# vfmatzkin/ct-unet

Hardware: AMD Instinct MI355X
Metric: voxels/sec fwd+bwd, 128^3 fp32 patch (higher is better)
Workload: dtype f32

## Files before the change

ct-unet_amd/csrc/conv3d.hip:

```cpp
#include "common.h"
#include "pack.h"
#include "bn_tail.h"

#ifndef CTU_K3S_OCC
#define CTU_K3S_OCC 2
#endif
#ifndef CTU_K3S_ALL
#define CTU_K3S_ALL 1
#endif
#ifndef CTU_WG_OCC
#define CTU_WG_OCC 2
#endif
#ifndef CTU_WG_BLOCKS
#define CTU_WG_BLOCKS 512
#endif

namespace {

typedef float gv2f __attribute__((ext_vector_type(2)));

struct ConvP {
    const float* in;
    const float* in_scale;
    const float* in_shift;
    const float* wp;
    const float* bias;
    float* out;
    float* stats;
    int in_cs, rin_p, in_relu, out_cs, nout_p, nbias;
    int N, D, H, W;
    int tiles_d, tiles_h, tiles_w;
    int n16;
    ctu_bn_tail tail;
};


__host__ __device__ inline void pick_tile(int W, int* td, int* th, int* tw) {
    if (W >= 16) { *td = 4; *th = 4; *tw = 16; }
    else if (W >= 8) { *td = 4; *th = 8; *tw = 8; }
    else { *td = 4; *th = 4; *tw = 4; }
}



template <int KS, int NT, int TD, int TH, int TW, int CCH = 1>
__global__ __launch_bounds__(256) void conv3d_fwd_kernel(ConvP p) {
    constexpr int PAD = (KS - 1) / 2;
    constexpr int HD = TD + KS - 1, HH = TH + KS - 1, HW = TW + KS - 1;
    constexpr int HV = HD * HH * HW;
    constexpr int NVOX = TD * TH * TW;
    constexpr int NMT = NVOX / 16;
    static_assert(NMT % 4 == 0, "block tile must hold a multiple of 4 M-tiles");
    constexpr int MT = NMT / 4;
    constexpr int STAPS = Taps<KS>::STAPS, NSTAGE = Taps<KS>::NSTAGE;
    constexpr int WFL = STAPS * NT * 128;
    constexpr int VSL = 8 * CCH + 4;
    constexpr int AQ = 2 * CCH;
    constexpr int AITEMS = HV * AQ;
    constexpr int AITER = (AITEMS + 255) / 256;
    static_assert(CCH == 1 || NSTAGE == 1, "multi-chunk staging needs all taps' weights in LDS at once");

    __shared__ __attribute__((aligned(16))) float sA[HV * VSL];
    __shared__ __attribute__((aligned(16))) float sW[CCH * WFL];
    __shared__ float sRed[4 * NT * 16 * 2];

    const int tid = threadIdx.x;
    const int lane = tid & 63, wave = tid >> 6;
// ... 1468 lines not shown
    int kw;
    bool ok = true;
    if (SM == 1 && SN == 1) kw = q;
    else if (SM == 2 && SN == 2) { kw = sm + sn; ok = !(sm == 0 && sn == 1); }
    else if (SN == 2) { if (q == 0) { kw = 0; ok = sn == 0; } else kw = 1 + sn; }
    else { if (q == 0) kw = sm; else { kw = 2; ok = sm == 1; } }
    const int cig = pair % n_ci_g, cog = pair / n_ci_g;
    const int cip = cig * CM + cil, co = cog * CN + col;
    const int ci = (cip < cin_p) ? (cinv ? cinv[cip] : (cip < Ci ? cip : -1)) : -1;
    if (ok && ci >= 0 && co < Co) dw[((size_t)co * Ci + ci) * 27 + r * 3 + kw] = tot;
}

struct K3sGeom { int sm, sn, tw, ntiles, n_ci_g, pairs, gx, tpb, nmf; };
static K3sGeom k3s_geom(int N, int D, int H, int W, int cin_p, int cout_p) {
    K3sGeom g;
    g.sm = cin_p == 8 ? 2 : 1; g.sn = cout_p == 8 ? 2 : 1;
    g.tw = (g.sm == 2 && g.sn == 2) ? 16 : 8;
    g.nmf = (g.sm == 2 && g.sn == 2) ? 9 : ((g.sm == 1 && g.sn == 1) ? 27 : 18);
    g.ntiles = N * ceil_div(D, 4) * ceil_div(H, 4) * ceil_div(W, g.tw);
    g.n_ci_g = ceil_div(cin_p, 16 / g.sm);
    g.pairs = g.n_ci_g * ceil_div(cout_p, 16 / g.sn);
    g.gx = wgrad_gx(g.ntiles, g.pairs);
    if (g.ntiles / g.gx < 4) {
        g.gx = (CTU_WG_BLOCKS / 2) / g.pairs;
        if (g.gx < 1) g.gx = 1;
        if (g.gx > g.ntiles) g.gx = g.ntiles;
    }
    g.tpb = ceil_div(g.ntiles, g.gx);
    g.gx = ceil_div(g.ntiles, g.tpb);
    return g;
}

static bool k3s_lazy_ok(int D, int H, int W, int k, int cin_p, int cout_p) {
    if (!use_k3s(k, W, cin_p, cout_p)) return false;
    const int sm = cin_p == 8 ? 2 : 1, sn = cout_p == 8 ? 2 : 1, tw = (sm == 2 && sn == 2) ? 16 : 8;
    return D % 4 == 0 && H % 4 == 0 && W % tw == 0 && cin_p % (16 / sm) == 0 && cout_p % (16 / sn) == 0;
}

template <int SM, int SN>
static int launch_wgrad_k3s(WgP p, float* dw, int Co, int Ci, const int32_t* cinv, hipStream_t st) {
    const K3sGeom g = k3s_geom(p.N, p.D, p.H, p.W, p.cin_p, p.cout_p);
    p.tiles_d = ceil_div(p.D, 4); p.tiles_h = ceil_div(p.H, 4); p.tiles_w = ceil_div(p.W, g.tw);
    p.ntiles = g.ntiles;
    p.n_ci_t = g.n_ci_g;
    if (p.lz_y) conv3d_wgrad_k3s_kernel<SM, SN, 0, true><<<dim3(g.gx, g.pairs), 256, 0, st>>>(p, g.tpb);
    else conv3d_wgrad_k3s_kernel<SM, SN><<<dim3(g.gx, g.pairs), 256, 0, st>>>(p, g.tpb);
    CTU_CHECK_LAUNCH("conv3d_wgrad_k3s");
    conv3d_wgrad_k3s_reduce_kernel<SM, SN><<<dim3(ceil_div(g.nmf * 256, 64), g.pairs), 64 * RPARTS, 0, st>>>(
        p.ws, dw, Co, Ci, cinv, p.cin_p, p.n_ci_t, g.gx);
    CTU_CHECK_LAUNCH("conv3d_wgrad_k3s_reduce");
    return CTU_OK;
}

template <int SM, int SN>
__global__ __launch_bounds__(256, 2) void conv3d_wgrad_k5s_kernel(WgP p, int tiles_per_block) {
    constexpr int UP = 0, PAD = 2;
    const int kd = blockIdx.z;
    constexpr int TD = 4, TH = 4, TW = (SM == 2 && SN == 2) ? 16 : 8, HD = TD, HH = TH + 2 * PAD, HW = TW + 2 * PAD, HV = HD * HH * HW;
    constexpr int KPR = TW / 4, NKS = TH * KPR;
    constexpr int CM = 16 / SM, CN = 16 / SN;
    constexpr int GW = TW + (SN - 1), GV = TD * TH * GW;
    constexpr int QN = (SM == 2 && SN == 2) ? 2 : ((SM == 1 && SN == 1) ? 5 : (SN == 2 ? 4 : 3));
    constexpr int NMF = 5 * QN;
    constexpr int AQ = CM / 4, GQ = CN / 4;
    constexpr int AITEMS = HV * AQ, AITER = (AITEMS + 255) / 256;
    constexpr int GITEMS = GV * GQ, GITER = (GITEMS + 255) / 256;

    constexpr int SAF = AITER * 256 * 4, SGF = GITER * 256 * 4;
    static_assert(SAF >= HV * CM && SGF >= GV * CN, "stage size");
    __shared__ __attribute__((aligned(16))) float sA[2 * SAF];
    __shared__ __attribute__((aligned(16))) float sG[2 * SGF];

    const int tid = threadIdx.x, lane = tid & 63, wave = tid >> 6;
    const int i = lane & 15, kq = lane >> 4;
    const int cig = blockIdx.y % p.n_ci_t, cog = UP ? (blockIdx.y / p.n_ci_t) % p.n_co_t : blockIdx.y / p.n_ci_t;
    const int par = UP ? blockIdx.y / (p.n_ci_t * p.n_co_t) : 0;
    const int pz = UP == 2 ? (par >> 1) & 1 : (par >> 2) & 1, py = UP == 2 ? par & 1 : (par >> 1) & 1, px = UP == 2 ? 0 : par & 1;
    const int gH = UP ? 2 * p.H : p.H, gW = UP ? 2 * p.W : p.W, gs = UP ? 2 : 1;
    const int ci0 = cig * CM, co0 = cog * CN;
    const bool has_xf = p.in_scale != nullptr;

    f32x4 acc[NMF];
#pragma unroll
    for (int t = 0; t < NMF; ++t) acc[t] = f32x4{0.f, 0.f, 0.f, 0.f};

    const int aq = tid % AQ, gq = tid % GQ;
    const bool a_ok = (ci0 + aq * 4) < p.cin_p, g_ok = (co0 + gq * 4) < p.cout_p;
    float4 sc = make_float4(1.f, 1.f, 1.f, 1.f), sh = make_float4(0.f, 0.f, 0.f, 0.f);
    if (has_xf && a_ok) {
        sc = *reinterpret_cast<const float4*>(p.in_scale + ci0 + aq * 4);
        sh = *reinterpret_cast<const float4*>(p.in_shift + ci0 + aq * 4);
    }
    const int xf_relu = has_xf ? p.in_relu : 0;
    const int boff = (SN == 2) ? ((i < 8) ? i : i - 16) : i;

    int tile = blockIdx.x * tiles_per_block;
    const int tile_end = min(p.ntiles, tile + tiles_per_block);
    float4 va[AITER], vg[GITER];

    unsigned aoff[AITER], goff[GITER];
    constexpr int FPW = 5;
    unsigned fw[(AITER + FPW - 1) / FPW], gw0 = 0;
#pragma unroll
    for (int q = 0; q < (AITER + FPW - 1) / FPW; ++q) fw[q] = 0;
#pragma unroll
    for (int it = 0; it < AITER; ++it) {
// ... 339 lines not shown
        g.tpb = ceil_div(g.ntiles, g.gx);
        g.gx = ceil_div(g.ntiles, g.tpb);
        return g;
    }
    g.nmf = 8;
    g.ntiles = N * ceil_div(D, 4) * ceil_div(H, 4) * ceil_div(W, 8);
    g.n_ci_g = ceil_div(cin_p, 16);
    g.n_co_g = ceil_div(nout_p, 16);
    g.pairs = 8 * g.n_ci_g * g.n_co_g;
    g.gx = wgrad_gx(g.ntiles, g.pairs);
    if (g.ntiles / g.gx < 4) {
        g.gx = (CTU_WG_BLOCKS / 2) / g.pairs;
        if (g.gx < 1) g.gx = 1;
        if (g.gx > g.ntiles) g.gx = g.ntiles;
    }
    g.tpb = ceil_div(g.ntiles, g.gx);
    g.gx = ceil_div(g.ntiles, g.tpb);
    return g;
}

}

static bool use_persist5(int k, int nt, int tw, int N, int D, int H, int W) {
    return k == 5 && tw == 16 && nt <= 2 && (long)N * ceil_div(D, 4) * ceil_div(H, 4) * ceil_div(W, 16) >= 256;
}

extern "C" int ctu_conv3d_layout(int k, int nout_p, int W) {
    return ((k == 3 || k == 5) && nout_p == 8 && W >= 32) ? 1 : 0;
}

extern "C" const char* ctu_conv3d_fwd_kernel_name(int N, int D, int H, int W, int k, int nout_p, int layout) {
    static thread_local char buf[64];
    if (layout == 1) return k == 3 ? "conv3d_fwd_k3_persist<1, true>" : "conv3d_fwd_k5_persist<1, true>";
    int nt, td, th, tw;
    pick_launch(N, D, H, W, k, nout_p, &nt, &td, &th, &tw);
    if (use_persist5(k, nt, tw, N, D, H, W)) snprintf(buf, sizeof(buf), "conv3d_fwd_k5_persist<%d, false>", nt);
    else if (k == 3 && tw == 16 && nt <= 2) snprintf(buf, sizeof(buf), "conv3d_fwd_k3_persist<%d, false>", nt);
    else snprintf(buf, sizeof(buf), "conv3d_fwd_kernel<%d, %d, %d, %d, %d>", k, nt, td, th, tw);
    return buf;
}

extern "C" const char* ctu_conv3d_wgrad_kernel_name(int W, int k, int cin_p, int cout_p) {
    static thread_local char buf[64];
    if (use_k3s(k, W, cin_p, cout_p))
        snprintf(buf, sizeof(buf), "conv3d_wgrad_k3s_kernel<%d, %d>", cin_p == 8 ? 2 : 1, cout_p == 8 ? 2 : 1);
    else if (use_k5s(k, W, cin_p, cout_p))
        snprintf(buf, sizeof(buf), "conv3d_wgrad_k5s_kernel<%d, %d>", cin_p == 8 ? 2 : 1, cout_p == 8 ? 2 : 1);
    else {
        int td, th, tw;
        pick_tile(W, &td, &th, &tw);
        snprintf(buf, sizeof(buf), "conv3d_wgrad_kernel<%d, %d, %d, %d, %d>", k, k == 3 ? 3 : 1, td, th, tw);
    }
    return buf;
}

extern "C" size_t ctu_conv3d_packed_floats(int k, int rin_p, int nout_p, int layout) {
    if ((k != 3 && k != 5) || rin_p <= 0 || nout_p <= 0) return 0;
    if (layout == 1) return nout_p == 8 ? (size_t)(rin_p / 8) * k * k * (k + 1) * 128 : 0;
    return (size_t)(rin_p / 8) * k * k * k * ceil_div(nout_p, 16) * 128;
}

static void persist_grid(int ntiles, int ny, int blocks_per_cu, int* gx, int* tpb) {
    int g = (256 * blocks_per_cu) / ny;
    if (g < 1) g = 1;
    if (g > ntiles) g = ntiles;
    *tpb = ceil_div(ntiles, g);
    *gx = ceil_div(ntiles, *tpb);
}

static bool use_persist(int k, int nt, int tw) { return k == 3 && tw == 16 && nt <= 2; }

extern "C" int ctu_conv3d_num_blocks(int N, int D, int H, int W, int k, int nout_p, int layout) {
    int gx, tpb;
    if (layout == 1) {
        persist_grid(N * ceil_div(D, 4) * ceil_div(H, 4) * ceil_div(W, 32), 1, k == 3 ? 2 : 1, &gx, &tpb);
        return gx;
    }
    int nt, td, th, tw;
    pick_launch(N, D, H, W, k, nout_p, &nt, &td, &th, &tw);
    const int ntiles = N * ceil_div(D, td) * ceil_div(H, th) * ceil_div(W, tw);
    if (use_persist5(k, nt, tw, N, D, H, W)) {
        persist_grid(ntiles, ceil_div(ceil_div(nout_p, 16), nt), 1, &gx, &tpb);
        return gx;
    }
    if (use_persist(k, nt, tw)) {
        persist_grid(ntiles, ceil_div(ceil_div(nout_p, 16), nt), nt == 1 ? CTU_FWD_OCC1 : 2, &gx, &tpb);
        return gx;
    }
    return ntiles;
}

extern "C" int ctu_pack_conv3d_weight(const float* w, float* wp, int Co, int Ci, int k, const int32_t* cinv,
                                      int rin_p, int nout_p, int mode, int layout, void* stream) {
    CTU_REQUIRE(k == 3 || k == 5, "pack_conv3d_weight: k=%d unsupported (3 or 5)", k);
    CTU_REQUIRE(rin_p % 8 == 0 && nout_p % 8 == 0, "pack_conv3d_weight: padded channels must be multiples of 8");
    CTU_REQUIRE(w && wp && Co > 0 && Ci > 0, "pack_conv3d_weight: null/empty argument");
    CTU_REQUIRE(layout == 0 || (layout == 1 && nout_p == 8), "pack_conv3d_weight: layout %d needs nout_p=8", layout);
    hipStream_t st = (hipStream_t)stream;
    if (layout == 1) {
        const int tot = (int)ctu_conv3d_packed_floats(k, rin_p, nout_p, 1);
        if (k == 3) pack_conv_w_pair8_kernel<3><<<ceil_div(tot, 256), 256, 0, st>>>(w, wp, Co, Ci, cinv, rin_p / 8, mode);
        else pack_conv_w_pair8_kernel<5><<<ceil_div(tot, 256), 256, 0, st>>>(w, wp, Co, Ci, cinv, rin_p / 8, mode);
        CTU_CHECK_LAUNCH("pack_conv3d_weight(pair8)");
        return CTU_OK;
    }
    const int n16 = ceil_div(nout_p, 16);
// ... 183 lines not shown
}

struct LazyBn { const float* y; const float* scale; const float* shift; const float* coef; float* out; int cp; };

static int conv3d_wgrad_impl(const float* in, int in_cs, int cin_p, const float* in_scale, const float* in_shift,
                             int in_relu, const float* gout, int g_cs, int cout_p, float* dw, float* dbias, int Co,
                             int Ci, const int32_t* cinv, float* ws, int N, int D, int H, int W, int k, const LazyBn* lz,
                             void* stream);

extern "C" int ctu_conv3d_wgrad(const float* in, int in_cs, int cin_p, const float* in_scale, const float* in_shift,
                                int in_relu, const float* gout, int g_cs, int cout_p, float* dw, float* dbias, int Co,
                                int Ci, const int32_t* cinv, float* ws, int N, int D, int H, int W, int k,
                                void* stream) {
    return conv3d_wgrad_impl(in, in_cs, cin_p, in_scale, in_shift, in_relu, gout, g_cs, cout_p, dw, dbias, Co, Ci, cinv, ws,
                             N, D, H, W, k, nullptr, stream);
}

extern "C" int ctu_conv3d_wgrad_bn_supported(int N, int D, int H, int W, int k, int cin_p, int cout_p) {
    return (N > 0 && k3s_lazy_ok(D, H, W, k, cin_p, cout_p)) ? 1 : 0;
}

extern "C" int ctu_conv3d_wgrad_bn(const float* in, int in_cs, int cin_p, const float* in_scale, const float* in_shift,
                                   int in_relu, const float* ga, int g_cs, int cout_p, const float* y,
                                   const float* bn_scale, const float* bn_shift, const float* coef, float* gy_out,
                                   float* dw, int Co, int Ci, const int32_t* cinv, float* ws, int N, int D, int H, int W,
                                   int k, void* stream) {
    CTU_REQUIRE(y && bn_scale && bn_shift && coef && gy_out, "conv3d_wgrad_bn: null pointer");
    CTU_REQUIRE(k3s_lazy_ok(D, H, W, k, cin_p, cout_p), "conv3d_wgrad_bn: geometry not supported (ask ctu_conv3d_wgrad_bn_supported)");
    CTU_REQUIRE(((uintptr_t)y & 15) == 0 && ((uintptr_t)gy_out & 15) == 0 && gy_out != ga, "conv3d_wgrad_bn: y / gy_out alignment, gy_out must not alias ga");
    const LazyBn lz = {y, bn_scale, bn_shift, coef, gy_out, cout_p};
    return conv3d_wgrad_impl(in, in_cs, cin_p, in_scale, in_shift, in_relu, ga, g_cs, cout_p, dw, nullptr, Co, Ci, cinv, ws,
                             N, D, H, W, k, &lz, stream);
}

static int conv3d_wgrad_impl(const float* in, int in_cs, int cin_p, const float* in_scale, const float* in_shift,
                             int in_relu, const float* gout, int g_cs, int cout_p, float* dw, float* dbias, int Co,
                             int Ci, const int32_t* cinv, float* ws, int N, int D, int H, int W, int k, const LazyBn* lz,
                             void* stream) {
    CTU_REQUIRE(k == 3 || k == 5, "conv3d_wgrad: k=%d unsupported (3 or 5)", k);
    CTU_REQUIRE(in && gout && dw && ws, "conv3d_wgrad: null pointer");
    CTU_REQUIRE(cin_p % 8 == 0 && cout_p % 8 == 0 && cin_p > 0 && cout_p > 0, "conv3d_wgrad: padded channels");
    CTU_REQUIRE(in_cs >= cin_p && in_cs % 4 == 0 && g_cs >= cout_p && g_cs % 4 == 0, "conv3d_wgrad: bad stride");
    CTU_REQUIRE(Co <= cout_p && Co > 0 && Ci > 0 && cin_p <= 256, "conv3d_wgrad: Co/Ci");
    CTU_REQUIRE(((uintptr_t)in & 15) == 0 && ((uintptr_t)gout & 15) == 0, "conv3d_wgrad: 16-byte alignment");
    hipStream_t st = (hipStream_t)stream;
    WgP p;
    p.in = in; p.in_scale = in_scale; p.in_shift = in_shift; p.g = gout; p.ws = ws;
    p.in_cs = in_cs; p.cin_p = cin_p; p.in_relu = in_relu; p.g_cs = g_cs; p.cout_p = cout_p;
    p.N = N; p.D = D; p.H = H; p.W = W;
    p.lz_y = nullptr; p.lz_out = nullptr; p.lz_scale = nullptr; p.lz_shift = nullptr; p.lz_coef = nullptr; p.lz_cp = 0;
    if (lz) { p.lz_y = lz->y; p.lz_out = lz->out; p.lz_scale = lz->scale; p.lz_shift = lz->shift; p.lz_coef = lz->coef; p.lz_cp = lz->cp; }
    int gz, gx, bt;
    wgrad_geom(N, D, H, W, k, cin_p, cout_p, &p.ntiles, &p.n_ci_t, &p.n_co_t, &gz, &gx, &bt);
    if (use_k3s(k, W, cin_p, cout_p)) {
        int rc2;
        if (cin_p == 8 && cout_p == 8) rc2 = launch_wgrad_k3s<2, 2>(p, dw, Co, Ci, cinv, st);
        else if (cout_p == 8) rc2 = launch_wgrad_k3s<1, 2>(p, dw, Co, Ci, cinv, st);
        else if (cin_p == 8) rc2 = launch_wgrad_k3s<2, 1>(p, dw, Co, Ci, cinv, st);
        else rc2 = launch_wgrad_k3s<1, 1>(p, dw, Co, Ci, cinv, st);
        if (rc2 != CTU_OK) return rc2;
        if (dbias) return ctu_channel_sum(gout, g_cs, cout_p, (int64_t)N * D * H * W, ws, dbias, Co, stream);
        return CTU_OK;
    }
    if (use_k5s(k, W, cin_p, cout_p)) {
        CTU_REQUIRE((int64_t)((4 + 2 * 2) * H + 8) * W * in_cs * 4 < (int64_t)1 << 31, "conv3d_wgrad: volume too large for 32-bit offsets");
        int rc2;
        if (cin_p == 8 && cout_p == 8) rc2 = launch_wgrad_k5s<2, 2>(p, dw, Co, Ci, cinv, st);
        else if (cout_p == 8) rc2 = launch_wgrad_k5s<1, 2>(p, dw, Co, Ci, cinv, st);
        else rc2 = launch_wgrad_k5s<2, 1>(p, dw, Co, Ci, cinv, st);
        if (rc2 != CTU_OK) return rc2;
        if (dbias) return ctu_channel_sum(gout, g_cs, cout_p, (int64_t)N * D * H * W, ws, dbias, Co, stream);
        return CTU_OK;
    }
    int rc = (k == 3) ? launch_wgrad<3, 3>(p, dw, Co, Ci, cinv, gz, gx, st)
                      : launch_wgrad<5, 1>(p, dw, Co, Ci, cinv, gz, gx, st);
    if (rc != CTU_OK) return rc;
    if (dbias) return ctu_channel_sum(gout, g_cs, cout_p, (int64_t)N * D * H * W, ws, dbias, Co, stream);
    return CTU_OK;
}

extern "C" size_t ctu_upconv_fused_wgrad_ws_floats(int N, int D, int H, int W, int cin_p, int nout_p) {
    const UpWgGeom a = upwg_geom(N, D, H, W, cin_p, nout_p, false), b = upwg_geom(N, D, H, W, cin_p, nout_p, true);
    const size_t na = (size_t)a.pairs * a.gx * a.nmf * 256, nb = (size_t)b.pairs * b.gx * b.nmf * 256;
    return na > nb ? na : nb;
}

static int upconv_fused_wgrad_impl(const float* in, int in_cs, int cin_p, const float* in_scale, const float* in_shift,
                                   int in_relu, const float* gout, int g_cs, int nout_p, float* dweff, float* ws,
                                   int N, int D, int H, int W, const LazyBn* lz, void* stream);

extern "C" int ctu_upconv_fused_wgrad(const float* in, int in_cs, int cin_p, const float* in_scale, const float* in_shift,
                                      int in_relu, const float* gout, int g_cs, int nout_p, float* dweff, float* ws,
                                      int N, int D, int H, int W, void* stream) {
    return upconv_fused_wgrad_impl(in, in_cs, cin_p, in_scale, in_shift, in_relu, gout, g_cs, nout_p, dweff, ws, N, D, H, W,
                                   nullptr, stream);
}

extern "C" int ctu_upconv_fused_wgrad_bn_supported(int N, int D, int H, int W, int cin_p, int nout_p) {
    return (N > 0 && D % 4 == 0 && H % 4 == 0 && W % 8 == 0 && cin_p % 16 == 0 && nout_p % 8 == 0) ? 1 : 0;
}

extern "C" int ctu_upconv_fused_wgrad_bn(const float* in, int in_cs, int cin_p, const float* in_scale, const float* in_shift,
                                         int in_relu, const float* ga, int g_cs, int nout_p, const float* y,
                                         const float* bn_scale, const float* bn_shift, const float* coef, float* gy_out,
                                         float* dweff, float* ws, int N, int D, int H, int W, void* stream) {
    CTU_REQUIRE(y && bn_scale && bn_shift && coef && gy_out, "upconv_fused_wgrad_bn: null pointer");
// ... 44 lines not shown
```

ct-unet_amd/ctunet_amd/_lib.py:

```python
from __future__ import annotations

import ctypes as C
import os

_HERE = os.path.dirname(os.path.abspath(__file__))
LIB_PATH = os.environ.get("CTUNET_HIP_LIB") or os.path.join(_HERE, "libctunet_hip.so")

P = C.c_void_p
I = C.c_int
L = C.c_int64
F = C.c_float
D = C.c_double
Z = C.c_size_t
U = C.c_uint64

class PackJob(C.Structure):
    _fields_ = [("w", C.c_void_p), ("wp", C.c_void_p), ("cinv", C.c_void_p), ("kind", C.c_int), ("Co", C.c_int),
                ("Ci", C.c_int), ("k", C.c_int), ("rin_p", C.c_int), ("nout_p", C.c_int), ("mode", C.c_int),
                ("layout", C.c_int)]


class BnTail(C.Structure):
    _fields_ = [("gamma", C.c_void_p), ("beta", C.c_void_p), ("running_mean", C.c_void_p), ("running_var", C.c_void_p),
                ("scale", C.c_void_p), ("shift", C.c_void_p), ("mean", C.c_void_p), ("invstd", C.c_void_p),
                ("num_batches_tracked", C.c_void_p), ("counter", C.c_void_p), ("count", C.c_double),
                ("momentum", C.c_float), ("eps", C.c_float), ("C", C.c_int), ("n_updates", C.c_int)]


class BnBwdTail(C.Structure):
    _fields_ = [("gamma", C.c_void_p), ("invstd", C.c_void_p), ("dgamma", C.c_void_p), ("dbeta", C.c_void_p),
                ("coef", C.c_void_p), ("mean", C.c_void_p), ("running_mean", C.c_void_p), ("running_var", C.c_void_p),
                ("num_batches_tracked", C.c_void_p), ("counter", C.c_void_p), ("count", C.c_double),
                ("momentum", C.c_float), ("eps", C.c_float), ("C", C.c_int)]


SIGNATURES = {
    "ctu_last_error": (C.c_char_p, []),
    "ctu_abi_version": (I, []),
    "ctu_arch": (C.c_char_p, []),
    "ctu_ncdhw_to_ndhwc": (I, [P, P, I, I, I, I, I, I, I, P]),
    "ctu_ndhwc_to_ncdhw": (I, [P, P, I, I, I, I, I, I, P]),
    "ctu_conv3d_layout": (I, [I, I, I]),
    "ctu_conv3d_fwd_kernel_name": (C.c_char_p, [I, I, I, I, I, I, I]),
    "ctu_conv3d_wgrad_kernel_name": (C.c_char_p, [I, I, I, I]),
    "ctu_conv3d_packed_floats": (Z, [I, I, I, I]),
    "ctu_conv3d_num_blocks": (I, [I, I, I, I, I, I, I]),
    "ctu_pack_conv3d_weight": (I, [P, P, I, I, I, P, I, I, I, I, P]),
    "ctu_pack_batch": (I, [P, I, P]),
    "ctu_conv3d_fwd": (I, [P, I, I, P, P, I, P, P, I, P, I, I, P, I, I, I, I, I, I, P, P]),
    "ctu_conv3d_wgrad_ws_floats": (Z, [I, I, I, I, I, I, I]),
    "ctu_conv3d_wgrad": (I, [P, I, I, P, P, I, P, I, I, P, P, I, I, P, P, I, I, I, I, I, P]),
    "ctu_conv3d_wgrad_bn_supported": (I, [I, I, I, I, I, I, I]),
    "ctu_conv3d_wgrad_bn": (I, [P, I, I, P, P, I, P, I, I, P, P, P, P, P, P, I, I, P, P, I, I, I, I, I, P]),
    "ctu_conv3d_first_supported": (I, [I, I, I, I]),
    "ctu_conv3d_first_num_blocks": (I, [I, I, I, I]),
    "ctu_conv3d_first_fwd": (I, [P, I, P, P, I, P, I, I, P, I, I, I, I, P, P]),
    "ctu_conv3d_first_bwd_data": (I, [P, I, P, I, I, P, I, I, I, I, P]),
    "ctu_conv3d_first_wgrad_ws_floats": (Z, [I, I, I, I, I]),
    "ctu_conv3d_first_wgrad": (I, [P, I, P, I, P, I, P, I, I, I, I, P]),
    "ctu_conv3d_first_wgrad_bn": (I, [P, I, P, I, P, P, P, P, P, P, I, P, I, I, I, I, P]),
    "ctu_bn_finalize": (I, [P, I, I, I, D, P, P, P, P, F, F, I, P, P, P, P, P, P]),
    "ctu_bn_eval_affine": (I, [P, P, P, P, F, I, I, P, P, P]),
    "ctu_bn_bwd_num_blocks": (I, [L]),
    "ctu_bn_relu_bwd_reduce": (I, [P, I, P, I, I, P, P, P, P, L, P, P, P]),
    "ctu_bn_bwd_finalize": (I, [P, I, I, I, D, P, P, P, P, P, P, P, P, F, F, P, P]),
    "ctu_bn_relu_bwd_apply": (I, [P, I, P, I, I, P, P, P, P, P, L, P]),
    "ctu_maxpool2_fwd": (I, [P, I, I, P, P, I, P, I, I, I, I, I, P]),
    "ctu_maxpool2_bwd": (I, [P, I, I, P, P, I, P, I, P, I, I, I, I, I, I, P]),
    "ctu_maxpool2_bwd_bn_num_blocks": (I, [I, I, I, I, I]),
    "ctu_maxpool2_bwd_bn": (I, [P, I, I, P, P, P, P, P, I, P, I, I, I, I, I, I, P, P, P]),
    "ctu_convt_packed_floats": (Z, [I, I]),
    "ctu_pack_convt_weight": (I, [P, P, I, I, P, I, I, I, P]),
    "ctu_convt2_fwd": (I, [P, I, I, P, P, I, P, P, I, P, I, I, I, I, I, I, P]),
    "ctu_convt2_bwd_data": (I, [P, I, I, P, P, I, I, I, I, I, I, P]),
    "ctu_convt2_wgrad_ws_floats": (Z, [I, I, I, I, I, I]),
    "ctu_convt2_wgrad": (I, [P, I, I, P, P, I, P, I, I, P, P, I, I, P, P, I, I, I, I, P]),
    "ctu_head_fwd": (I, [P, I, I, P, P, I, P, P, P, I, I, I, I, P, P, I, L, P]),
    "ctu_head_bwd_ws_floats": (Z, [I, L, I, I]),
    "ctu_head_bwd": (I, [P, I, I, P, P, I, P, P, P, I, I, I, I, P, P, P, I, P, P, P, I, L, P]),
    "ctu_head_bwd_num_blocks": (I, [I, L]),
    "ctu_head_bwd_bn": (I, [P, I, I, P, P, I, P, P, P, I, I, I, I, P, P, P, I, P, P, P, I, L, P, P, I, P, P, P]),
    "ctu_loss_ws_floats": (Z, [I, L]),
    "ctu_loss_fwd": (I, [P, P, I, L, F, F, I, P, P, P]),
    "ctu_loss_bwd": (I, [P, P, I, L, F, F, I, P, P, P, P, I, P]),
    "ctu_skip_add": (I, [P, I, P, P, I, P, I, P, P, I, P, I, I, L, P]),
    "ctu_upconv_fused_supported": (I, [I, I, I, I, I, I]),
    "ctu_upconv_fused_packed_floats": (Z, [I, I]),
    "ctu_upconv_fused_num_blocks": (I, [I, I, I, I, I]),
    "ctu_upconv_fused_pack_ws_floats": (Z, [I, I]),
    "ctu_upconv_fused_pack": (I, [P, P, P, I, I, P, I, I, P, P, P, P]),
    "ctu_upconv_fused_fwd": (I, [P, I, I, P, P, I, P, P, P, I, I, P, I, I, I, I, P, P]),
    "ctu_upconv_fused_wgrad_ws_floats": (Z, [I, I, I, I, I, I]),
    "ctu_upconv_fused_wgrad": (I, [P, I, I, P, P, I, P, I, I, P, P, I, I, I, I, P]),
    "ctu_upconv_fused_wgrad_bn_supported": (I, [I, I, I, I, I, I]),
    "ctu_upconv_fused_wgrad_bn": (I, [P, I, I, P, P, I, P, I, I, P, P, P, P, P, P, P, I, I, I, I, P]),
    "ctu_upconv_fused_project_ws_floats": (Z, [I, L]),
    "ctu_upconv_fused_project": (I, [P, P, I, I, I, I, I, I, P, P, P, I, I, I, P, P, P, P, P]),
# ... 113 lines not shown
```

ct-unet_amd/ctunet_amd/ops.py:

```python
from __future__ import annotations

import os

from dataclasses import dataclass
from typing import Optional, Tuple

import torch

from . import _lib


def pad8(c: int) -> int:
    return (c + 7) // 8 * 8


LP_CODE = {torch.bfloat16: 1, torch.float16: 2}
ACT_DTYPES = (torch.float32, torch.bfloat16, torch.float16)


def _need_cuda(t: torch.Tensor, name: str) -> None:
    if not t.is_cuda:
        raise RuntimeError(f"ctunet_amd: {name} must live on the GPU (MI355X); this path has no CPU fallback")
    if t.dtype != torch.float32 and t.dtype != torch.int32:
        raise RuntimeError(f"ctunet_amd: {name} must be float32, got {t.dtype}")
# ... 272 lines not shown
    if x.lp:
        assert out.dtype == x.dtype and wp.dtype == x.dtype, (x.dtype, out.dtype, wp.dtype)
        t0 = TIMER.begin() if TIMER is not None else None
        _lib.check(lib.ctu_lp_conv3d_fwd(x.lp, x.ptr, x.cs, x.cp, _ptr(x.scale), _ptr(x.shift), int(x.relu), wp.data_ptr(),
                                         _ptr(bias), 0 if bias is None else bias.numel(), out.ptr, out.cs, out.cp,
                                         _ptr(stats), n, d, h, w, k, layout, _tail_arg(tail), _stream()), "lp_conv3d_fwd")
        if t0 is not None:
            ci, co = algo_ch if algo_ch is not None else (x.cp, out.cp)
            vox = n * d * h * w
            name = lib.ctu_lp_conv3d_fwd_kernel_name(n, d, h, w, k, x.cp, out.cp, layout).decode()
            TIMER.end(f"{name}<{'bf16' if x.lp == 1 else 'f16'}, {k}>", 2.0 * ci * co * k ** 3 * vox, 2.0 * vox * (ci + co), t0,
                      (w, x.cp, out.cp))
        return
    t0 = TIMER.begin() if TIMER is not None else None
    _lib.check(lib.ctu_conv3d_fwd(x.ptr, x.cs, x.cp, _ptr(x.scale), _ptr(x.shift), int(x.relu), wp.data_ptr(),
                                  _ptr(bias), 0 if bias is None else bias.numel(), out.ptr, out.cs, out.cp, _ptr(stats),
                                  n, d, h, w, k, layout, _tail_arg(tail), _stream()), "conv3d_fwd")
    if t0 is not None:
        ci, co = algo_ch if algo_ch is not None else (x.cp, out.cp)
        vox = n * d * h * w
        TIMER.end(lib.ctu_conv3d_fwd_kernel_name(n, d, h, w, k, out.cp, layout).decode(), 2.0 * ci * co * k ** 3 * vox,
                  4.0 * vox * (ci + co), t0, (w, x.cp, out.cp))


def conv3d_wgrad(x: CL, g: CL, co: int, ci: int, k: int, cinv: Optional[torch.Tensor], ws: torch.Tensor,
                 want_bias: bool) -> Tuple[torch.Tensor, Optional[torch.Tensor]]:
    n, d, h, w = x.dims
    lib = _lib.load()
    if x.lp:
        assert g.dtype == x.dtype
        need = lib.ctu_lp_conv3d_wgrad_ws_floats(n, d, h, w, k, x.cp, g.cp)
        assert ws.numel() >= need, (ws.numel(), need)
        dw = torch.empty((co, ci, k, k, k), dtype=torch.float32, device=x.buf.device)
        t0 = TIMER.begin() if TIMER is not None else None
        _lib.check(lib.ctu_lp_conv3d_wgrad(x.lp, x.ptr, x.cs, x.cp, _ptr(x.scale), _ptr(x.shift), int(x.relu), g.ptr, g.cs,
                                           g.cp, dw.data_ptr(), co, ci, _ptr(cinv), ws.data_ptr(), n, d, h, w, k, _stream()),
                   "lp_conv3d_wgrad")
        if t0 is not None:
            vox = n * d * h * w
            name = lib.ctu_lp_conv3d_wgrad_kernel_name(d, h, w, k, x.cp, g.cp).decode()
            TIMER.end(f"{name}<{'bf16' if x.lp == 1 else 'f16'}, {k}> (+slab reduce)",
                      2.0 * ci * co * k ** 3 * vox, 2.0 * vox * (ci + co), t0, (w, x.cp, g.cp))
        return dw, (channel_sum(g, co) if want_bias else None)
    need = lib.ctu_conv3d_wgrad_ws_floats(n, d, h, w, k, x.cp, g.cp)
    assert ws.numel() >= need, (ws.numel(), need)
    dw = torch.empty((co, ci, k, k, k), dtype=torch.float32, device=x.buf.device)
    db = torch.empty(co, dtype=torch.float32, device=x.buf.device) if want_bias else None
    t0 = TIMER.begin() if TIMER is not None else None
    _lib.check(lib.ctu_conv3d_wgrad(x.ptr, x.cs, x.cp, _ptr(x.scale), _ptr(x.shift), int(x.relu), g.ptr, g.cs, g.cp,
                                    dw.data_ptr(), _ptr(db), co, ci, _ptr(cinv), ws.data_ptr(), n, d, h, w, k,
                                    _stream()), "conv3d_wgrad")
    if t0 is not None:
        vox = n * d * h * w
        TIMER.end(lib.ctu_conv3d_wgrad_kernel_name(w, k, x.cp, g.cp).decode() + " (+slab reduce)",
                  2.0 * ci * co * k ** 3 * vox, 4.0 * vox * (ci + co), t0, (w, x.cp, g.cp))
    return dw, db


def conv3d_wgrad_bn_supported(dims, k: int, cin_p: int, cout_p: int, dtype=torch.float32) -> bool:
    n, d, h, w = dims
    if lp(dtype):
        return bool(_lib.load().ctu_lp_conv3d_wgrad_bn_supported(n, d, h, w, k, cin_p, cout_p))
    return bool(_lib.load().ctu_conv3d_wgrad_bn_supported(n, d, h, w, k, cin_p, cout_p))


def conv3d_wgrad_bn(x: CL, ga: CL, y: CL, vec: torch.Tensor, coef: torch.Tensor, gy: CL, co: int, ci: int, k: int,
                    cinv: Optional[torch.Tensor], ws: torch.Tensor) -> torch.Tensor:
    n, d, h, w = x.dims
    lib = _lib.load()
    assert ga.dims == x.dims and y.dims == x.dims and gy.dims == x.dims and ga.dtype == x.dtype == y.dtype == gy.dtype
    assert y.cs == ga.cs == gy.cs and y.cp == ga.cp == gy.cp and gy.buf.data_ptr() != ga.buf.data_ptr()
    if x.lp:
        need = lib.ctu_lp_conv3d_wgrad_ws_floats(n, d, h, w, k, x.cp, ga.cp)
        assert ws.numel() >= need, (ws.numel(), need)
        dw = torch.empty((co, ci, k, k, k), dtype=torch.float32, device=x.buf.device)
        t0 = TIMER.begin() if TIMER is not None else None
        _lib.check(lib.ctu_lp_conv3d_wgrad_bn(x.lp, x.ptr, x.cs, x.cp, _ptr(x.scale), _ptr(x.shift), int(x.relu), ga.ptr, ga.cs,
                                              ga.cp, y.ptr, vec[0].data_ptr(), vec[1].data_ptr(), coef.data_ptr(), gy.ptr,
                                              dw.data_ptr(), co, ci, _ptr(cinv), ws.data_ptr(), n, d, h, w, k, _stream()),
                   "lp_conv3d_wgrad_bn")
        if t0 is not None:
            vox = n * d * h * w
            name = lib.ctu_lp_conv3d_wgrad_kernel_name(d, h, w, k, x.cp, ga.cp).decode()
            TIMER.end(f"{name}<{'bf16' if x.lp == 1 else 'f16'}, {k}> (+slab reduce)",
                      2.0 * ci * co * k ** 3 * vox, 2.0 * vox * (ci + co), t0, (w, x.cp, ga.cp))
        return dw
    need = lib.ctu_conv3d_wgrad_ws_floats(n, d, h, w, k, x.cp, ga.cp)
    assert ws.numel() >= need, (ws.numel(), need)
    dw = torch.empty((co, ci, k, k, k), dtype=torch.float32, device=x.buf.device)
    t0 = TIMER.begin() if TIMER is not None else None
    _lib.check(lib.ctu_conv3d_wgrad_bn(x.ptr, x.cs, x.cp, _ptr(x.scale), _ptr(x.shift), int(x.relu), ga.ptr, ga.cs, ga.cp,
                                       y.ptr, vec[0].data_ptr(), vec[1].data_ptr(), coef.data_ptr(), gy.ptr,
                                       dw.data_ptr(), co, ci, _ptr(cinv), ws.data_ptr(), n, d, h, w, k, _stream()),
               "conv3d_wgrad_bn")
    if t0 is not None:
        vox = n * d * h * w
        TIMER.end(lib.ctu_conv3d_wgrad_kernel_name(w, k, x.cp, ga.cp).decode() + " (+slab reduce)",
                  2.0 * ci * co * k ** 3 * vox, 4.0 * vox * (ci + co), t0, (w, x.cp, ga.cp))
    return dw


def conv3d_wgrad_ws(dims, k, cin_p, cout_p, dtype=torch.float32) -> int:
    n, d, h, w = dims
    if lp(dtype):
        return _lib.load().ctu_lp_conv3d_wgrad_ws_floats(n, d, h, w, k, cin_p, cout_p)
    return _lib.load().ctu_conv3d_wgrad_ws_floats(n, d, h, w, k, cin_p, cout_p)


def pack_conv_w_lp(w: torch.Tensor, cinv: Optional[torch.Tensor], rin_p: int, nout_p: int, mode: int, dtype: torch.dtype,
                   into: Optional[torch.Tensor] = None, layout: int = 0) -> torch.Tensor:
    _need_cuda(w, "conv weight")
    co, ci, k = w.shape[0], w.shape[1], w.shape[2]
    lib = _lib.load()
    n = lib.ctu_lp_conv3d_packed_elems(k, rin_p, nout_p)
    wp = into if into is not None else torch.empty(n, dtype=dtype, device=w.device)
    assert wp.numel() == n and wp.dtype == dtype
    _lib.check(lib.ctu_lp_pack_conv3d_weight(LP_CODE[dtype], w.contiguous().data_ptr(), wp.data_ptr(), co, ci, k, _ptr(cinv),
                                             rin_p, nout_p, mode, layout, _stream()), "lp_pack_conv3d_weight")
    return wp


def conv_first_supported(k: int, cin: int, nout_p: int, w: int) -> bool:
    return bool(_lib.load().ctu_conv3d_first_supported(k, cin, nout_p, w))


def conv_first_num_blocks(dims) -> int:
    n, d, h, w = dims
    return _lib.load().ctu_conv3d_first_num_blocks(n, d, h, w)


def conv_first_fwd(x: torch.Tensor, w: torch.Tensor, bias: Optional[torch.Tensor], out: CL,
                   stats: Optional[torch.Tensor], tail=None) -> None:
    _need_cuda(x, "input")
    n, cin, d, h, w_ = x.shape
    lib = _lib.load()
    t0 = TIMER.begin() if TIMER is not None else None
    _dual(out.lp, "conv3d_first_fwd", x.data_ptr(), cin, w.data_ptr(), _ptr(bias), 0 if bias is None else bias.numel(),
          out.ptr, out.cs, w.shape[0], _ptr(stats), n, d, h, w_, _tail_arg(tail), _stream())
    if t0 is not None:
        vox = n * d * h * w_
        TIMER.end(f"first_fwd_kernel<{cin}>", 2.0 * cin * w.shape[0] * 27 * vox, 4.0 * vox * (cin + w.shape[0]), t0)


def conv_first_bwd_data(g: CL, w: torch.Tensor, cin: int) -> torch.Tensor:
    n, d, h, w_ = g.dims
    dx = torch.empty((n, cin, d, h, w_), dtype=torch.float32, device=g.buf.device)
    lib = _lib.load()
    t0 = TIMER.begin() if TIMER is not None else None
    pair = bool(g.lp and g.cp == 8 and lib.ctu_lp_conv3d_first_bwd_data_pair_supported(cin, w_))
    if pair:
# ... 752 lines not shown
```

include/ctunet_hip.h:

```cpp
#ifndef CTUNET_HIP_H
#define CTUNET_HIP_H

#include <stddef.h>
#include <stdint.h>

#ifdef __cplusplus
extern "C" {
#endif

#define CTU_OK 0
#define CTU_EINVAL (-1)
#define CTU_ELAUNCH (-2)

#define CTU_F32 0
#define CTU_BF16 1
#define CTU_F16 2

typedef struct ctu_bn_tail {
    const float* gamma; const float* beta;
    float* running_mean; float* running_var;
    float* scale; float* shift; float* mean; float* invstd;
    long long* num_batches_tracked;
    unsigned int* counter;
    double count;
    float momentum, eps;
    int C, n_updates;
} ctu_bn_tail;
typedef struct ctu_bn_bwd_tail {
    const float* gamma; const float* invstd;
    float* dgamma; float* dbeta; float* coef;
    const float* mean; float* running_mean; float* running_var;
    long long* num_batches_tracked;
    unsigned int* counter;
    double count;
    float momentum, eps;
    int C;
} ctu_bn_bwd_tail;

const char* ctu_last_error(void);
int ctu_abi_version(void);
const char* ctu_arch(void);

int ctu_ncdhw_to_ndhwc(const float* src, float* dst, int N, int C, int D, int H, int W,
                       int cp, int cs, void* stream);
int ctu_ndhwc_to_ncdhw(const float* src, float* dst, int N, int C, int D, int H, int W,
                       int cs, void* stream);

int ctu_conv3d_layout(int k, int nout_p, int W);
const char* ctu_conv3d_fwd_kernel_name(int N, int D, int H, int W, int k, int nout_p, int layout);
const char* ctu_conv3d_wgrad_kernel_name(int W, int k, int cin_p, int cout_p);
size_t ctu_conv3d_packed_floats(int k, int rin_p, int nout_p, int layout);
int ctu_conv3d_num_blocks(int N, int D, int H, int W, int k, int nout_p, int layout);

int ctu_pack_conv3d_weight(const float* w, float* wp, int Co, int Ci, int k,
                           const int32_t* cinv, int rin_p, int nout_p, int mode, int layout,
                           void* stream);

typedef struct {
    const float* w;
    float* wp;
    const int32_t* cinv;
    int kind, Co, Ci, k, rin_p, nout_p, mode, layout;
} ctu_pack_job;
int ctu_pack_batch(const ctu_pack_job* jobs, int n, void* stream);

int ctu_conv3d_fwd(const float* in, int in_cs, int rin_p,
                   const float* in_scale, const float* in_shift, int in_relu,
                   const float* wp, const float* bias, int nbias,
                   float* out, int out_cs, int nout_p, float* stats,
                   int N, int D, int H, int W, int k, int layout, const ctu_bn_tail* tail, void* stream);

size_t ctu_conv3d_wgrad_ws_floats(int N, int D, int H, int W, int k, int cin_p, int cout_p);
int ctu_conv3d_wgrad(const float* in, int in_cs, int cin_p,
                     const float* in_scale, const float* in_shift, int in_relu,
                     const float* gout, int g_cs, int cout_p,
                     float* dw, float* dbias, int Co, int Ci, const int32_t* cinv,
                     float* ws, int N, int D, int H, int W, int k, void* stream);
int ctu_conv3d_wgrad_bn_supported(int N, int D, int H, int W, int k, int cin_p, int cout_p);
int ctu_conv3d_wgrad_bn(const float* in, int in_cs, int cin_p,
                        const float* in_scale, const float* in_shift, int in_relu,
                        const float* ga, int g_cs, int cout_p, const float* y,
                        const float* bn_scale, const float* bn_shift, const float* coef, float* gy_out,
                        float* dw, int Co, int Ci, const int32_t* cinv,
                        float* ws, int N, int D, int H, int W, int k, void* stream);

int ctu_conv3d_first_supported(int k, int cin, int nout_p, int W);
int ctu_conv3d_first_num_blocks(int N, int D, int H, int W);
int ctu_conv3d_first_fwd(const float* x, int cin, const float* w, const float* bias, int nbias,
                         float* out, int out_cs, int Co, float* stats,
                         int N, int D, int H, int W, const ctu_bn_tail* tail, void* stream);
int ctu_conv3d_first_bwd_data(const float* g, int g_cs, const float* w, int cin, int Co, float* dx,
                              int N, int D, int H, int W, void* stream);
size_t ctu_conv3d_first_wgrad_ws_floats(int N, int D, int H, int W, int cin);
int ctu_conv3d_first_wgrad(const float* x, int cin, const float* g, int g_cs, float* dw, int Co,
                           float* ws, int N, int D, int H, int W, void* stream);
int ctu_conv3d_first_wgrad_bn(const float* x, int cin, const float* ga, int g_cs, const float* y, const float* bn_scale,
                              const float* bn_shift, const float* coef, float* gy_out, float* dw, int Co, float* ws,
                              int N, int D, int H, int W, void* stream);

int ctu_bn_finalize(const float* stats, int nblocks, int C, int cp, double count,
                    const float* gamma, const float* beta,
                    float* running_mean, float* running_var, float momentum, float eps,
                    int n_updates, float* scale, float* shift, float* mean_out,
// ... 272 lines not shown
```

Measured before the change: 640.7 million.

## Add 32-wide plane-tiled wgrad kernel for k3 convs with 16x16 channel groups

```diff
diff --git a/ct-unet_amd/csrc/conv3d.hip b/ct-unet_amd/csrc/conv3d.hip
--- a/ct-unet_amd/csrc/conv3d.hip
+++ b/ct-unet_amd/csrc/conv3d.hip
@@ -13,6 +13,9 @@
 #endif
 #ifndef CTU_WG_BLOCKS
 #define CTU_WG_BLOCKS 512
+#endif
+#ifndef CTU_WG32
+#define CTU_WG32 1
 #endif
 
 namespace {
@@ -1587,6 +1590,238 @@
     return CTU_OK;
 }
 
+template <int SM, int SN, bool LZ>
+__global__ __launch_bounds__(256, 2) void wgrad32_plane_kernel(WgP p, int tiles_per_block) {
+    constexpr int TD = 4, TH = 4, TW = 32, HD = TD + 2, HH = TH + 2, HW = TW + 2, HV = HD * HH * HW;
+    constexpr int NKK = TW / 4;
+    constexpr int SW = (SM == 2 && SN == 2) ? 16 : 8, NSB = TW / SW, KPS = SW / 4;
+    constexpr int CM = 16 / SM, CN = 16 / SN;
+    constexpr int QN = (SM == 2 && SN == 2) ? 1 : ((SM == 1 && SN == 1) ? 3 : 2);
+    constexpr int NMF = 9 * QN;
+    constexpr int AQ = CM / 4, AITEMS = HV * AQ, AITER = (AITEMS + 255) / 256;
+    constexpr int FPW = 5;
+    __shared__ __attribute__((aligned(16))) float sA[HV * CM];
+
+    const int tid = threadIdx.x, lane = tid & 63, wave = tid >> 6;
+    const int i = lane & 15, kq = lane >> 4;
+    const int cig = blockIdx.y % p.n_ci_t, cog = blockIdx.y / p.n_ci_t;
+    const int ci0 = cig * CM, co0 = cog * CN;
+    const bool has_xf = p.in_scale != nullptr;
+
+    f32x4 acc[NMF];
+#pragma unroll
+    for (int t = 0; t < NMF; ++t) acc[t] = f32x4{0.f, 0.f, 0.f, 0.f};
+
+    const int aq = tid % AQ;
+    float4 sc = make_float4(1.f, 1.f, 1.f, 1.f), sh = make_float4(0.f, 0.f, 0.f, 0.f);
+    if (has_xf) {
+        sc = *reinterpret_cast<const float4*>(p.in_scale + ci0 + aq * 4);
+        sh = *reinterpret_cast<const float4*>(p.in_shift + ci0 + aq * 4);
+    }
+    const int xf_relu = has_xf ? p.in_relu : 0;
+    unsigned aoff[AITER], fw[(AITER + FPW - 1) / FPW];
+#pragma unroll
+    for (int q = 0; q < (AITER + FPW - 1) / FPW; ++q) fw[q] = 0;
+#pragma unroll
+    for (int it = 0; it < AITER; ++it) {
+        const int e = tid + it * 256, v = (e < AITEMS) ? e / AQ : 0;
+        const int pw = v % HW, t2 = v / HW, ph = t2 % HH, pd = t2 / HH;
+        aoff[it] = (unsigned)(((pd * p.H + ph) * p.W + pw) * p.in_cs + ci0 + aq * 4) * 4u;
+        const unsigned face = (pd == 0 ? 1u : 0u) | (pd == HD - 1 ? 2u : 0u) | (ph == 0 ? 4u : 0u) | (ph == HH - 1 ? 8u : 0u) |
+                              (pw == 0 ? 16u : 0u) | (pw == HW - 1 ? 32u : 0u);
+        fw[it / FPW] |= face << (6 * (it % FPW));
+    }
+    const unsigned safe_a = (unsigned)(((p.H + 1) * p.W + 1) * p.in_cs + ci0 + aq * 4) * 4u;
+
+    const int sp = (SN == 2) ? (i >> 3) : 0, col = (SN == 2) ? (i & 7) : i;
+    const unsigned g_lane = (unsigned)((kq - sp + 1) * p.g_cs + co0 + col) * 4u;
+    const unsigned g_kk = 16u * p.g_cs, g_w0 = (unsigned)(p.g_cs + co0 + col) * 4u;
+    float l_sc = 0.f, l_sh = 0.f, l_k0 = 0.f, l_A = 0.f, l_B = 0.f;
+    if constexpr (LZ) {
+        const int c = co0 + col;
+        l_sc = p.lz_scale[c]; l_sh = p.lz_shift[c];
+        l_k0 = p.lz_coef[c]; l_A = p.lz_coef[3 * p.lz_cp + c]; l_B = p.lz_coef[4 * p.lz_cp + c];
+    }
+    const bool gy_store = LZ && cig == 0 && sp == 0;
+
+    typedef const volatile __attribute__((address_space(3))) float* lds_f_ptr;
+    const lds_f_ptr vA = (lds_f_ptr)sA + ((wave * HH) * HW + kq) * CM + i;
+
+    struct Box { int tx, ty, tz, n; };
+    Box box;
+    int tile = blockIdx.x * tiles_per_block;
+    const int tile_end = min(p.ntiles, tile + tiles_per_block);
+    {
+        int t = tile;
+        box.tx = t % p.tiles_w; t /= p.tiles_w;
+        box.ty = t % p.tiles_h; t /= p.tiles_h;
+        box.tz = t % p.tiles_d; box.n = t / p.tiles_d;
+    }
+
+    for (; tile < tile_end; ++tile) {
+        const int d0 = box.tz * TD, h0 = box.ty * TH, w0 = box.tx * TW;
+        const long long org = (((long long)box.n * p.D + d0) * p.H + h0) * p.W + w0;
+        const char* abase = reinterpret_cast<const char*>(p.in + (org - ((long long)p.H * p.W + p.W + 1)) * p.in_cs);
+        const unsigned bface = (d0 == 0 ? 1u : 0u) | (d0 + TD == p.D ? 2u : 0u) | (h0 == 0 ? 4u : 0u) | (h0 + TH == p.H ? 8u : 0u) |
+                               (w0 == 0 ? 16u : 0u) | (w0 + TW == p.W ? 32u : 0u);
+
+        const long long prow = org - 1 + (long long)wave * p.H * p.W;
+        const bool w_lo = sp == 1 && kq == 0 && w0 == 0;
+        float bq[TH][NKK];
+        float yq[LZ ? TH : 1][LZ ? NKK : 1];
+#pragma unroll
+        for (int th = 0; th < TH; ++th) {
+            const long long ro = (prow + (long long)th * p.W) * p.g_cs;
+            const char* rb = reinterpret_cast<const char*>(p.g + ro);
+            const char* ry = reinterpret_cast<const char*>(LZ ? p.lz_y + ro : p.g);
+#pragma unroll
+            for (int kk = 0; kk < NKK; ++kk) {
+                const unsigned off = (kk == 0 && w_lo) ? g_w0 : g_lane + kk * g_kk;
+                bq[th][kk] = *reinterpret_cast<const float*>(rb + off);
+                if constexpr (LZ) yq[th][kk] = *reinterpret_cast<const float*>(ry + off);
+            }
+        }
+
+#pragma unroll
+        for (int th = 0; th < TH; ++th) {
+            char* rb = reinterpret_cast<char*>(p.lz_out + (prow + (long long)th * p.W) * p.g_cs);
+#pragma unroll
+            for (int kk = 0; kk < NKK; ++kk) {
+                float v = bq[th][kk];
+                if constexpr (LZ) {
+                    const float y = yq[th][kk];
+                    v = fmaf(l_k0, (fmaf(y, l_sc, l_sh) > 0.f) ? v : 0.f, fmaf(l_A, y, l_B));
+                    if (gy_store) *reinterpret_cast<float*>(rb + g_lane + kk * g_kk) = v;
+                }
+                if (kk == 0) v = w_lo ? 0.f : v;
+                bq[th][kk] = v;
+            }
+        }
+        constexpr int CH = 8;
+#pragma unroll
+        for (int c0 = 0; c0 < AITER; c0 += CH) {
+            float4 va[CH];
+#pragma unroll
+            for (int u = 0; u < CH; ++u) {
+                const int it = c0 + u;
+                if (it < AITER) {
+                    const bool ok = (fw[it / FPW] & (bface << (6 * (it % FPW)))) == 0u;
+                    va[u] = *reinterpret_cast<const float4*>(abase + (ok ? aoff[it] : safe_a));
+                }
+            }
+#pragma unroll
+            for (int u = 0; u < CH; ++u) {
+                const int it = c0 + u;
+                if (it < AITER && (it < AITER - 1 || tid + it * 256 < AITEMS)) {
+                    const bool ok = (fw[it / FPW] & (bface << (6 * (it % FPW)))) == 0u;
+                    const float4 t = xform4(va[u], sc, sh, xf_relu);
+                    *reinterpret_cast<float4*>(&sA[(tid + it * 256) * 4]) =
+                        make_float4(ok ? t.x : 0.f, ok ? t.y : 0.f, ok ? t.z : 0.f, ok ? t.w : 0.f);
+                }
+            }
+        }
+
+        __syncthreads();
+
+        {
+            constexpr int R = 8, NA = 3 * HH * NKK * QN;
+            auto a_read = [&](int j) -> float {
+                const int q = j % QN, kkl = (j / QN) % KPS, hr = (j / (QN * KPS)) % HH, sb = (j / (QN * KPS * HH)) % NSB,
+                          kd = j / (QN * KPS * HH * NSB);
+                return vA[((kd * HH + hr) * HW + 4 * (sb * KPS + kkl) + q) * CM];
+            };
+            float ar[R];
+#pragma unroll
+            for (int j = 0; j < R; ++j) ar[j] = a_read(j);
+            static_assert(R == 8, "fake-use list");
+            asm volatile("" : "+v"(ar[0]), "+v"(ar[1]), "+v"(ar[2]), "+v"(ar[3]), "+v"(ar[4]), "+v"(ar[5]), "+v"(ar[6]), "+v"(ar[7]));
+#pragma unroll
+            for (int kd = 0; kd < 3; ++kd)
+#pragma unroll
+            for (int sb = 0; sb < NSB; ++sb)
+#pragma unroll
+            for (int hr = 0; hr < HH; ++hr)
+#pragma unroll
+            for (int kkl = 0; kkl < KPS; ++kkl)
+#pragma unroll
+            for (int q = 0; q < QN; ++q) {
+                const int j = (((kd * NSB + sb) * HH + hr) * KPS + kkl) * QN + q, kk = sb * KPS + kkl;
+#pragma unroll
+                for (int kh = 0; kh < 3; ++kh) {
+                    const int th = hr - kh;
+                    if (th >= 0 && th < TH) {
+                        const int t = (kd * 3 + kh) * QN + q;
+                        acc[t] = __builtin_amdgcn_mfma_f32_16x16x4f32(ar[j % R], bq[th][kk], acc[t], 0, 0, 0);
+                        __builtin_amdgcn_sched_group_barrier(0x008, 1, 0);
+                    }
+                }
+                if (j + R < NA) {
+                    ar[j % R] = a_read(j + R);
+                    __builtin_amdgcn_sched_group_barrier(0x100, 1, 0);
+                }
+            }
+        }
+        __syncthreads();
+        if (++box.tx == p.tiles_w) { box.tx = 0; if (++box.ty == p.tiles_h) { box.ty = 0; if (++box.tz == p.tiles_d) { box.tz = 0; ++box.n; } } }
+    }
+
+    constexpr int RT = (HV * CM / 1024) < NMF ? (HV * CM / 1024) : NMF;
+    static_assert(RT >= 1, "reduction scratch");
+    const size_t slab = (size_t)blockIdx.y * gridDim.x + blockIdx.x;
+    float* dst = p.ws + slab * (NMF * 256);
+    for (int t0 = 0; t0 < NMF; t0 += RT) {
+        __syncthreads();
+#pragma unroll
+        for (int t = 0; t < NMF; ++t)
+            if (t >= t0 && t < t0 + RT) {
+#pragma unroll
+                for (int r = 0; r < 4; ++r) sA[(wave * RT + (t - t0)) * 256 + (kq * 4 + r) * 16 + i] = acc[t][r];
+            }
+        __syncthreads();
+        const int nt = (NMF - t0) < RT ? (NMF - t0) : RT;
+        for (int e = tid; e < nt * 256; e += 256)
+            dst[t0 * 256 + e] = (sA[e] + sA[RT * 256 + e]) + (sA[2 * RT * 256 + e] + sA[3 * RT * 256 + e]);
+    }
+}
+
+struct Wg32Geom { K3sGeom g; int ntiles, tpb; };
+static bool wg32_geom(int N, int D, int H, int W, int k, int cin_p, int cout_p, Wg32Geom* out) {
+    if (!CTU_WG32 || k != 3 || N <= 0 || W < 32 || W % 32 != 0 || D % 4 != 0 || H % 4 != 0) return false;
+    if (!use_k3s(k, W, cin_p, cout_p)) return false;
+    const int cm = cin_p == 8 ? 8 : 16, cn = cout_p == 8 ? 8 : 16;
+    if (cin_p % cm != 0 || cout_p % cn != 0) return false;
+    if (CTU_WG32 == 1 && !(cm == 16 && cn == 16 && (cin_p / 16) * (cout_p / 16) >= 4)) return false;
+    const K3sGeom g = k3s_geom(N, D, H, W, cin_p, cout_p);
+    const int r = 32 / g.tw;
+    if (g.tpb % r != 0) return false;
+    out->g = g;
+    out->ntiles = g.ntiles / r;
+    out->tpb = g.tpb / r;
+    return true;
+}
+
+template <int SM, int SN>
+static int launch_wgrad32(WgP p, const Wg32Geom& w, float* dw, int Co, int Ci, const int32_t* cinv, hipStream_t st) {
+    const K3sGeom& g = w.g;
+    p.tiles_d = p.D / 4; p.tiles_h = p.H / 4; p.tiles_w = p.W / 32;
+    p.ntiles = w.ntiles;
+    p.n_ci_t = g.n_ci_g;
+    if (p.lz_y) wgrad32_plane_kernel<SM, SN, true><<<dim3(g.gx, g.pairs), 256, 0, st>>>(p, w.tpb);
+    else wgrad32_plane_kernel<SM, SN, false><<<dim3(g.gx, g.pairs), 256, 0, st>>>(p, w.tpb);
+    CTU_CHECK_LAUNCH("wgrad32_plane");
+    conv3d_wgrad_k3s_reduce_kernel<SM, SN><<<dim3(ceil_div(g.nmf * 256, 64), g.pairs), 64 * RPARTS, 0, st>>>(
+        p.ws, dw, Co, Ci, cinv, p.cin_p, p.n_ci_t, g.gx);
+    CTU_CHECK_LAUNCH("conv3d_wgrad_k3s_reduce");
+    return CTU_OK;
+}
+
+static int launch_wgrad32_any(WgP p, const Wg32Geom& w, float* dw, int Co, int Ci, const int32_t* cinv, hipStream_t st) {
+    if (p.cin_p == 8 && p.cout_p == 8) return launch_wgrad32<2, 2>(p, w, dw, Co, Ci, cinv, st);
+    if (p.cin_p == 8) return launch_wgrad32<2, 1>(p, w, dw, Co, Ci, cinv, st);
+    if (p.cout_p == 8) return launch_wgrad32<1, 2>(p, w, dw, Co, Ci, cinv, st);
+    return launch_wgrad32<1, 1>(p, w, dw, Co, Ci, cinv, st);
+}
+
 template <int SM, int SN>
 __global__ __launch_bounds__(256, 2) void conv3d_wgrad_k5s_kernel(WgP p, int tiles_per_block) {
     constexpr int UP = 0, PAD = 2;
@@ -2032,6 +2267,16 @@
         snprintf(buf, sizeof(buf), "conv3d_wgrad_kernel<%d, %d, %d, %d, %d>", k, k == 3 ? 3 : 1, td, th, tw);
     }
     return buf;
+}
+
+extern "C" const char* ctu_conv3d_wgrad_kernel_name_dims(int N, int D, int H, int W, int k, int cin_p, int cout_p) {
+    static thread_local char buf[64];
+    Wg32Geom wg;
+    if (wg32_geom(N, D, H, W, k, cin_p, cout_p, &wg)) {
+        snprintf(buf, sizeof(buf), "wgrad32_plane_kernel<%d, %d>", cin_p == 8 ? 2 : 1, cout_p == 8 ? 2 : 1);
+        return buf;
+    }
+    return ctu_conv3d_wgrad_kernel_name(W, k, cin_p, cout_p);
 }
 
 extern "C" size_t ctu_conv3d_packed_floats(int k, int rin_p, int nout_p, int layout) {
@@ -2321,6 +2566,13 @@
     if (lz) { p.lz_y = lz->y; p.lz_out = lz->out; p.lz_scale = lz->scale; p.lz_shift = lz->shift; p.lz_coef = lz->coef; p.lz_cp = lz->cp; }
     int gz, gx, bt;
     wgrad_geom(N, D, H, W, k, cin_p, cout_p, &p.ntiles, &p.n_ci_t, &p.n_co_t, &gz, &gx, &bt);
+    Wg32Geom wg;
+    if (wg32_geom(N, D, H, W, k, cin_p, cout_p, &wg)) {
+        const int rc2 = launch_wgrad32_any(p, wg, dw, Co, Ci, cinv, st);
+        if (rc2 != CTU_OK) return rc2;
+        if (dbias) return ctu_channel_sum(gout, g_cs, cout_p, (int64_t)N * D * H * W, ws, dbias, Co, stream);
+        return CTU_OK;
+    }
     if (use_k3s(k, W, cin_p, cout_p)) {
         int rc2;
         if (cin_p == 8 && cout_p == 8) rc2 = launch_wgrad_k3s<2, 2>(p, dw, Co, Ci, cinv, st);
diff --git a/ct-unet_amd/ctunet_amd/_lib.py b/ct-unet_amd/ctunet_amd/_lib.py
--- a/ct-unet_amd/ctunet_amd/_lib.py
+++ b/ct-unet_amd/ctunet_amd/_lib.py
@@ -43,6 +43,7 @@
     "ctu_conv3d_layout": (I, [I, I, I]),
     "ctu_conv3d_fwd_kernel_name": (C.c_char_p, [I, I, I, I, I, I, I]),
     "ctu_conv3d_wgrad_kernel_name": (C.c_char_p, [I, I, I, I]),
+    "ctu_conv3d_wgrad_kernel_name_dims": (C.c_char_p, [I, I, I, I, I, I, I]),
     "ctu_conv3d_packed_floats": (Z, [I, I, I, I]),
     "ctu_conv3d_num_blocks": (I, [I, I, I, I, I, I, I]),
     "ctu_pack_conv3d_weight": (I, [P, P, I, I, I, P, I, I, I, I, P]),
diff --git a/ct-unet_amd/ctunet_amd/ops.py b/ct-unet_amd/ctunet_amd/ops.py
--- a/ct-unet_amd/ctunet_amd/ops.py
+++ b/ct-unet_amd/ctunet_amd/ops.py
@@ -348,7 +348,7 @@
                                     _stream()), "conv3d_wgrad")
     if t0 is not None:
         vox = n * d * h * w
-        TIMER.end(lib.ctu_conv3d_wgrad_kernel_name(w, k, x.cp, g.cp).decode() + " (+slab reduce)",
+        TIMER.end(lib.ctu_conv3d_wgrad_kernel_name_dims(n, d, h, w, k, x.cp, g.cp).decode() + " (+slab reduce)",
                   2.0 * ci * co * k ** 3 * vox, 4.0 * vox * (ci + co), t0, (w, x.cp, g.cp))
     return dw, db
 
@@ -391,7 +391,7 @@
                "conv3d_wgrad_bn")
     if t0 is not None:
         vox = n * d * h * w
-        TIMER.end(lib.ctu_conv3d_wgrad_kernel_name(w, k, x.cp, ga.cp).decode() + " (+slab reduce)",
+        TIMER.end(lib.ctu_conv3d_wgrad_kernel_name_dims(n, d, h, w, k, x.cp, ga.cp).decode() + " (+slab reduce)",
                   2.0 * ci * co * k ** 3 * vox, 4.0 * vox * (ci + co), t0, (w, x.cp, ga.cp))
     return dw
 
diff --git a/include/ctunet_hip.h b/include/ctunet_hip.h
--- a/include/ctunet_hip.h
+++ b/include/ctunet_hip.h
@@ -49,6 +49,7 @@
 int ctu_conv3d_layout(int k, int nout_p, int W);
 const char* ctu_conv3d_fwd_kernel_name(int N, int D, int H, int W, int k, int nout_p, int layout);
 const char* ctu_conv3d_wgrad_kernel_name(int W, int k, int cin_p, int cout_p);
+const char* ctu_conv3d_wgrad_kernel_name_dims(int N, int D, int H, int W, int k, int cin_p, int cout_p);
 size_t ctu_conv3d_packed_floats(int k, int rin_p, int nout_p, int layout);
 int ctu_conv3d_num_blocks(int N, int D, int H, int W, int k, int nout_p, int layout);
 
```

Result: no change. 640.5 million (median of 6 runs) (-0.0%).
